# lturing/tacotronv2_wavernn_chinese

Measured on AMD Instinct MI355X. Metric: audio ksamples/sec (22.05 kHz, 10-bit RAW WaveRNN, batch=1 per GPU), higher is better.
Workload: dtype f32

## Files before the change

tacotronv2_wavernn_chinese_amd/csrc/loop_team2.hip:

```cpp
#include "team_common.h"

#define T2_THREADS 512

namespace {

template <int N>
__device__ __forceinline__ void peek_n(const u64 *base, unsigned idx, unsigned stride, u64 (&g)[N]) {
#pragma unroll
    for (int i = 0; i < N; ++i) g[i] = __hip_atomic_load(base + idx + (unsigned)i * stride, __ATOMIC_RELAXED, __HIP_MEMORY_SCOPE_AGENT);
}
template <int N, int SHIFT>
__device__ __forceinline__ bool tags_ok(const u64 (&g)[N], unsigned tag) {
    bool ok = true;
#pragma unroll
    for (int i = 0; i < N; ++i) ok = ok && ((unsigned)(g[i] >> SHIFT) == tag);
    return ok;
}
template <int N, int SHIFT>
__device__ __forceinline__ void finish_n(const u64 *base, unsigned idx, unsigned stride, unsigned tag, u64 (&g)[N], bool &dead,
                                         unsigned *err, unsigned code) {
    unsigned spins = 0;
    while (!dead && !__all(tags_ok<N, SHIFT>(g, tag))) {
        if (++spins > TEAM_SPIN_MAX) { dead = true; if ((threadIdx.x & 63) == 0) atomicExch(err, code); break; }
        peek_n<N>(base, idx, stride, g);
    }
}

#ifndef T2_HOIST_LDS
#define T2_HOIST_LDS 1
#endif
#ifndef T2_STRAIGHT_POLL
#define T2_STRAIGHT_POLL 7
#endif
#ifndef T2_DEFER_OUT
#define T2_DEFER_OUT 0
#endif
#ifndef T2_PRESLEEP
#define T2_PRESLEEP 0
#endif

__device__ __forceinline__ void hoist_fence() {
#if T2_HOIST_LDS
    __builtin_amdgcn_sched_barrier(0);
#endif
}
__device__ __forceinline__ void pin(float &v) {
#if T2_HOIST_LDS
    asm volatile("" : "+v"(v));
#endif
}

#if T2_STRAIGHT_POLL & 1
__device__ __forceinline__ unsigned take_granule(const u64 *base, unsigned idx, unsigned tag, bool &dead, unsigned *err, unsigned code) {
#if T2_PRESLEEP
    __builtin_amdgcn_s_sleep(T2_PRESLEEP);
#endif
    u64 g;
    for (unsigned spins = 0;;) {
        g = __hip_atomic_load(base + idx, __ATOMIC_RELAXED, __HIP_MEMORY_SCOPE_AGENT);
        if (__all((unsigned)(g >> 32) == tag) || dead) break;
        if (++spins > TEAM_SPIN_MAX) { dead = true; if ((threadIdx.x & 63) == 0) atomicExch(err, code); break; }
    }
    return (unsigned)g;
}
#else
__device__ __forceinline__ unsigned take_granule(const u64 *base, unsigned idx, unsigned tag, bool &dead, unsigned *err, unsigned code) {
    u64 ga[1];
#if T2_PRESLEEP
    __builtin_amdgcn_s_sleep(T2_PRESLEEP);
#endif
    peek_n<1>(base, idx, 1, ga);
    finish_n<1, 32>(base, idx, 1, tag, ga, dead, err, code);
    return (unsigned)ga[0];
}
#endif

__device__ __forceinline__ float rows_max(float v) {
    asm volatile(
        "s_nop 1\n\t"
        "v_max_f32_dpp %0, %0, %0 row_bcast:15 row_mask:0xa bank_mask:0xf\n\t"
        "s_nop 1\n\t"
        "v_max_f32_dpp %0, %0, %0 row_bcast:31 row_mask:0xc bank_mask:0xf\n\t"
        "s_nop 1"
        : "+v"(v));
    return v;
}

typedef unsigned u4 __attribute__((ext_vector_type(4)));
#ifndef T2_RACE_SLEEP
#define T2_RACE_SLEEP 3
#endif
__device__ __forceinline__ u4 race_load(const u64 *base, unsigned off) {
    u4 g;
    asm volatile("global_load_dwordx4 %0, %1, %2 sc1\n\t"
                 "s_waitcnt vmcnt(0)"
                 : "=&v"(g) : "v"(off), "s"(base) : "memory");
    return g;
}
__device__ __forceinline__ bool race_ok(const u4 &g, unsigned tag) { return (g.y >> 10) == tag && (g.w >> 10) == tag; }

#define XB_PLANE 68
#define XB_VEC (8 * XB_PLANE)
__device__ __forceinline__ int perm(int j) { return ((j >> 2) & 7) * XB_PLANE + (j >> 5) * 4 + (j & 3); }

typedef float f2 __attribute__((ext_vector_type(2)));
__device__ __forceinline__ f2 mk2(float a, float b) { f2 r; r.x = a; r.y = b; return r; }
__device__ __forceinline__ f2 pkfma(f2 a, f2 b, f2 c) { return __builtin_elementwise_fma(a, b, c); }

__device__ __forceinline__ void dot32x3(const float *w, const float *vec, int q, float &o0, float &o1, float &o2) {
    const float4 *p = (const float4 *)vec + q;
    f2 a = mk2(0.f, 0.f), b = mk2(0.f, 0.f), c = mk2(0.f, 0.f);
#pragma unroll
    for (int h = 0; h < 2; ++h) {
        float4 x[4];
#pragma unroll
        for (int k = 0; k < 4; ++k) x[k] = p[(4 * h + k) * (XB_PLANE / 4)];
#pragma unroll
        for (int k = 0; k < 4; ++k) {
            const int kk = 4 * h + k;
            const f2 xl = mk2(x[k].x, x[k].y), xh = mk2(x[k].z, x[k].w);
            a = pkfma(mk2(w[4 * kk + 0], w[4 * kk + 1]), xl, a);
            b = pkfma(mk2(w[32 + 4 * kk + 0], w[32 + 4 * kk + 1]), xl, b);
            c = pkfma(mk2(w[64 + 4 * kk + 0], w[64 + 4 * kk + 1]), xl, c);
            a = pkfma(mk2(w[4 * kk + 2], w[4 * kk + 3]), xh, a);
            b = pkfma(mk2(w[32 + 4 * kk + 2], w[32 + 4 * kk + 3]), xh, b);
            c = pkfma(mk2(w[64 + 4 * kk + 2], w[64 + 4 * kk + 3]), xh, c);
        }
    }
    o0 = a.x + a.y; o1 = b.x + b.y; o2 = c.x + c.y;
}
__device__ __forceinline__ void dot32x3_mixed(const float *w, const float4 *wl_, const float *vec, int q, float &o0, float &o1, float &o2) {
    const float4 *p = (const float4 *)vec + q;
    f2 a = mk2(0.f, 0.f), b = mk2(0.f, 0.f), c = mk2(0.f, 0.f);
#pragma unroll
    for (int h = 0; h < 2; ++h) {
        float4 x[4], wn[4];
#pragma unroll
        for (int k = 0; k < 4; ++k) { x[k] = p[(4 * h + k) * (XB_PLANE / 4)]; wn[k] = wl_[(4 * h + k) * 256]; }
#pragma unroll
        for (int k = 0; k < 4; ++k) {
            const int kk = 4 * h + k;
            const f2 xl = mk2(x[k].x, x[k].y), xh = mk2(x[k].z, x[k].w);
            a = pkfma(mk2(w[4 * kk + 0], w[4 * kk + 1]), xl, a);
            b = pkfma(mk2(w[32 + 4 * kk + 0], w[32 + 4 * kk + 1]), xl, b);
            c = pkfma(mk2(wn[k].x, wn[k].y), xl, c);
            a = pkfma(mk2(w[4 * kk + 2], w[4 * kk + 3]), xh, a);
            b = pkfma(mk2(w[32 + 4 * kk + 2], w[32 + 4 * kk + 3]), xh, b);
            c = pkfma(mk2(wn[k].z, wn[k].w), xh, c);
        }
    }
    o0 = a.x + a.y; o1 = b.x + b.y; o2 = c.x + c.y;
}
__device__ __forceinline__ float dot32(const float *w, const float *vec, int q) {
    const float4 *p = (const float4 *)vec + q;
    f2 s0 = mk2(0.f, 0.f), s1 = mk2(0.f, 0.f);
    float4 x[8];
#pragma unroll
    for (int k = 0; k < 8; ++k) x[k] = p[k * (XB_PLANE / 4)];
#pragma unroll
    for (int k = 0; k < 8; ++k) {
        s0 = pkfma(mk2(w[4 * k + 0], w[4 * k + 1]), mk2(x[k].x, x[k].y), s0);
        s1 = pkfma(mk2(w[4 * k + 2], w[4 * k + 3]), mk2(x[k].z, x[k].w), s1);
    }
    return (s0.x + s0.y) + (s1.x + s1.y);
}

constexpr int L_COND = 0;
constexpr int L_CSTA = L_COND + 512 * 4;
constexpr int L_GH1 = L_CSTA + 512 * 4;
constexpr int L_CSTQ = L_GH1 + 1536;
constexpr int L_HAND = L_CSTQ + 256;
constexpr int L_MISC = L_HAND + 128;
constexpr int L_XB = L_MISC + 64;
constexpr int XB_H1 = 0, XB_X2 = 1, XB_X3 = 2, XB_H2 = 3, XB_F1 = 4, XB_F2 = 5;
constexpr int L_SW = L_XB + 6 * XB_VEC;
constexpr int L_FC3 = L_SW + 8 * 256 * 4;
constexpr int L_XTAB = L_FC3 + 16384;
constexpr int L_TOTAL = L_XTAB + 1024;
static_assert(L_TOTAL * 4 <= 163840, "LDS budget");
constexpr int M_XF = 9;

constexpr unsigned G_X3 = 0, G_F1 = 1024, G_F2 = 2048, G_PR = 3072, G_GH = 4096;

}

#define P2(i)                                                               \
    do {                                                                    \
        if (PROF) {                                                         \
            const u64 now_ = __builtin_readcyclecounter();                  \
            prof_acc[i] += now_ - prof_last;                                \
            prof_last = now_;                                               \
        }                                                                   \
    } while (0)

template <int MODE, bool PROF, bool RAGGED>
__global__ void __launch_bounds__(T2_THREADS, 2) loop_team2_kernel(WrnnTeamArgs a) {
    extern __shared__ __attribute__((aligned(16))) char smem[];
    float *lds = (float *)smem;
    float *xb = lds + L_XB;
    float *gh1s = lds + L_GH1;
    int *misc_i = (int *)(lds + L_MISC);
    float *misc_f = lds + L_MISC;

    const int tid = threadIdx.x;
    const int lane = tid & 63, wave = __builtin_amdgcn_readfirstlane(tid >> 6);
    const bool isC = wave < 4;
    const int wl = wave & 3;
    if (isC) __builtin_amdgcn_s_setprio(3);
    const int r4 = lane >> 4, q = lane & 15;
    const WrnnDims d = a.d;
    const int NC = d.NC, HOP = d.HOP, T = a.T;
    const float4 *swl = (const float4 *)(lds + L_SW) + (tid - 256);

    int team, g;
    if (!join_team(a.ctl, a.err, misc_i, a.n_teams, team, g) || team >= a.n_rows) return;
    u64 *mail = a.mail + (size_t)team * WRNN_TEAM_MAIL_GRANULES;

    const int unit = 16 * g + 4 * wl + r4;
    const int qslot = wl * 4 + r4;
    const int c3row0 = 32 * g + 8 * wl + 2 * r4;
    const bool has_fc3 = c3row0 < NC;

    float wv[160];
    {
        const float *src = a.team_w + (size_t)g * WRNN_TEAM_NWREG * WRNN_TEAM_THREADS + (wl * 64 + lane);
        if (isC) {
#pragma unroll
            for (int i = 0; i < 96; ++i) wv[i] = src[(size_t)(96 + i) * WRNN_TEAM_THREADS];
#pragma unroll
            for (int i = 0; i < 64; ++i) wv[96 + i] = src[(size_t)(288 + i) * WRNN_TEAM_THREADS];
        } else {
#pragma unroll
            for (int i = 0; i < 96; ++i) wv[i] = src[(size_t)i * WRNN_TEAM_THREADS];
#pragma unroll
            for (int i = 0; i < 64; ++i) wv[96 + i] = src[(size_t)(192 + i) * WRNN_TEAM_THREADS];
#pragma unroll
            for (int k = 0; k < 8; ++k)
                ((float4 *)(lds + L_SW))[k * 256 + (tid - 256)] =
                    make_float4(src[(size_t)(256 + 4 * k) * WRNN_TEAM_THREADS], src[(size_t)(257 + 4 * k) * WRNN_TEAM_THREADS],
                                src[(size_t)(258 + 4 * k) * WRNN_TEAM_THREADS], src[(size_t)(259 + 4 * k) * WRNN_TEAM_THREADS]);
        }
        const float4 *f3 = (const float4 *)(a.team_fc3 + (size_t)g * 16384);
        float4 *dst = (float4 *)(lds + L_FC3);
        for (int i = tid; i < 4096; i += T2_THREADS) dst[i] = f3[i];
        if (MODE == WRNN_MODE_RAW)
            for (int k = tid; k < 1024; k += T2_THREADS) lds[L_XTAB + k] = 2.0f * (float)k / ((float)NC - 1.0f) - 1.0f;
        ((float4 *)(lds + L_CSTA))[tid] = make_float4(a.wI0[tid], a.u1[tid], a.u1[512 + tid], a.u1[1024 + tid]);
        if (!isC && q == 0) {
            float *cq = lds + L_CSTQ + qslot * 16;
            cq[0] = a.w[a.off.r1_bhh + unit]; cq[1] = a.w[a.off.r1_bhh + 512 + unit]; cq[2] = a.w[a.off.r1_bhh + 1024 + unit];
            cq[3] = a.w[a.off.r2_bhh + unit]; cq[4] = a.w[a.off.r2_bhh + 512 + unit]; cq[5] = a.w[a.off.r2_bhh + 1024 + unit];
            cq[6] = has_fc3 ? a.w[a.off.fc3_b + c3row0] : 0.0f;
            cq[7] = (c3row0 + 1 < NC) ? a.w[a.off.fc3_b + c3row0 + 1] : 0.0f;
        }
    }
    __syncthreads();
    float *cstQ = lds + L_CSTQ + qslot * 16;
    float *hand = lds + L_HAND + qslot * 8;
    const int pj = perm(tid), pu = perm(unit);
    const int sidx = tid - 256;

    bool dead = false;
    unsigned epoch = 0;
    u64 prof_acc[17] = {0};
    u64 prof_last = 0;

    for (int it = team; it < (RAGGED ? a.n_slots : a.n_rows); it += a.n_teams) {
        int row = it;
        if constexpr (RAGGED) {
            row = a.sched[it];
            if (row < 0) continue;
        }
        const WrnnRow rw = a.rows[row];
        uint64_t kseed = a.seed;
        uint32_t krow = (uint32_t)row;
        if (a.keys) { const WrnnRowKey k = a.keys[row]; kseed = k.seed; krow = k.row; }
        int64_t seg_end = a.seg0 + a.seg_len;
        if constexpr (RAGGED) {
            if (a.seg0 >= rw.steps) continue;
            if (seg_end > rw.steps) seg_end = rw.steps;
        }
        const bool resume = a.seg0 > 0;
        float *st = a.state + (size_t)row * WRNN_TEAM_STATE_FLOATS;
        const float4 *CONDg = (const float4 *)a.tabCOND + ((size_t)row * a.seg_len - (size_t)a.seg0) * 512;
        const float *C2g = a.tabC2 + (size_t)rw.utt * (T + 1) * 1536;
        const float *C3g = a.tabC3 + (size_t)rw.utt * (T + 1) * 512;
        const float *C4g = a.tabC4 + (size_t)rw.utt * (T + 1) * 512;

        float h1_j = resume ? st[tid] : 0.0f;
        float xfeed = resume ? st[4096] : (a.x_init ? a.x_init[row] : 0.0f);
        xb[XB_H2 * XB_VEC + pj] = resume ? st[512 + tid] : 0.0f;
        for (int i = tid; i < 1536; i += T2_THREADS) gh1s[i] = resume ? st[1024 + i] : a.w[a.off.r1_bhh + i];
        if (tid == 0) misc_f[M_XF] = xfeed;
        const int64_t pos0 = rw.start + a.seg0;
        int nfi = (int)(pos0 / HOP), nph = (int)(pos0 - (int64_t)nfi * HOP);
        int cst_frame = -1000000;
        int pend_frame = -1;
        float nzE0 = 0.f, nzE1 = 0.f, nzn0 = 0.f, nzn1 = 0.f;
        float4 cnext0 = make_float4(0.f, 0.f, 0.f, 0.f), cnext1 = cnext0;

        auto s_prepare = [&](int64_t ts, unsigned ep_of_ts) {
            const bool live = nfi < T;
            const int fi = live ? nfi : T;
            if (++nph == HOP) { nph = 0; ++nfi; }
            pend_frame = fi;
            ((float4 *)(lds + L_COND))[sidx] = cnext0;
            ((float4 *)(lds + L_COND))[sidx + 256] = cnext1;
        };
        auto s_prefetch = [&](int64_t ts) {
            if (ts < seg_end) {
                const float4 *cp = CONDg + (size_t)ts * 512;
                const unsigned so = (unsigned)sidx & 255u;
                cnext0 = cp[so];
                cnext1 = cp[256 + so];
            }
        };
        auto s_noise = [&](int64_t ts, unsigned ep_of_ts) {
            if (MODE == WRNN_MODE_MOL && wave == 4 && lane <= NC / 3) {
                const int nr = NC / 3;
                float u;
                if (a.noise_mode == WRNN_NOISE_INJECTED)
                    u = lane < nr ? a.noise1[((size_t)ts * a.n_rows + row) * nr + lane] : a.noise2[(size_t)ts * a.n_rows + row];
                else
                    u = wrnn_uniform_mol(kseed, (uint64_t)ts, krow, (uint32_t)lane);
                misc_f[32 + 16 * (ep_of_ts & 1u) + lane] = lane < nr ? -logf(-logf(u)) : logf(u) - logf(1.0f - u);
            }
            if (MODE == WRNN_MODE_RAW && has_fc3) {
                float nz0 = 0.f, nz1 = 0.f;
                if (a.noise_mode == WRNN_NOISE_INJECTED) {
                    const float *qp = a.noise1 + ((size_t)ts * a.n_rows + row) * NC + c3row0;
                    nz0 = -logf(qp[0]); nz1 = -logf(qp[1]);
                    if (q == 0) { hand[4 + 2 * (ep_of_ts & 1u)] = nz0; hand[5 + 2 * (ep_of_ts & 1u)] = nz1; }
                } else if (a.noise_mode == WRNN_NOISE_PHILOX) {
                    if ((ts & 31) == 0) {
                        const Philox4 pz = wrnn_raw_block(kseed, (uint64_t)ts + 2u * (unsigned)q, krow, (uint32_t)c3row0);
                        nzE0 = -__logf(-logf(u01_from_bits(pz.x)));
                        nzE1 = -__logf(-logf(u01_from_bits(pz.y)));
                        nzn0 = -__logf(-logf(u01_from_bits(pz.z)));
                        nzn1 = -__logf(-logf(u01_from_bits(pz.w)));
                    }
                    if (q == (int)((ts >> 1) & 15)) {
                        const bool odd = (ts & 1) != 0;
                        hand[4 + 2 * (ep_of_ts & 1u)] = odd ? nzn0 : nzE0;
                        hand[5 + 2 * (ep_of_ts & 1u)] = odd ? nzn1 : nzE1;
                    }
                } else if (q == 0) { hand[4 + 2 * (ep_of_ts & 1u)] = 0.f; hand[5 + 2 * (ep_of_ts & 1u)] = 0.f; }
            }
        };
        auto s_frame_consts = [&]() {
            if (pend_frame >= 0 && pend_frame != cst_frame) {
                if (q == 0) {
                    const int fi = pend_frame;
                    cstQ[8] = C2g[(size_t)fi * 1536 + unit]; cstQ[9] = C2g[(size_t)fi * 1536 + 512 + unit];
                    cstQ[10] = C2g[(size_t)fi * 1536 + 1024 + unit];
                    cstQ[11] = C3g[(size_t)fi * 512 + unit];
                    cstQ[12] = C4g[(size_t)fi * 512 + unit];
                }
                cst_frame = __builtin_amdgcn_readfirstlane(pend_frame);
            }
        };
        if (!isC) {
            if (q == 0) {
                hand[0] = resume ? st[2560 + unit] : cstQ[3];
                hand[1] = resume ? st[2560 + 512 + unit] : cstQ[4];
                hand[2] = resume ? st[2560 + 1024 + unit] : cstQ[5];
            }
            s_prefetch(a.seg0);
            s_prepare(a.seg0, epoch + 1);
            s_prefetch(a.seg0 + 1);
            s_noise(a.seg0, epoch + 1);
            s_frame_consts();
        }
        __syncthreads();

        int out_k = 0;
        float out_x = 0.0f;
        for (int64_t t = a.seg0; t < seg_end; ++t) {
            ++epoch;
            const unsigned par = epoch & 1u;
            if (PROF) prof_last = __builtin_readcyclecounter();

            float x2_j;
            {
                const float4 cA = ((const float4 *)(lds + L_CSTA))[tid];
                const float4 cd = ((const float4 *)(lds + L_COND))[tid];
                const float ghr = gh1s[tid], ghz = gh1s[512 + tid], ghn = gh1s[1024 + tid];
                const float xprev = xfeed;
                const float xin = fmaf(cA.x, xprev, cd.x);
                const float rg = sigmoid_fast(fmaf(cA.y, xprev, cd.y) + ghr);
                const float zg = sigmoid_fast(fmaf(cA.z, xprev, cd.z) + ghz);
                const float ng = tanh_fast(fmaf(cA.w, xprev, cd.w) + rg * ghn);
                h1_j = (1.0f - zg) * ng + zg * h1_j;
                x2_j = xin + h1_j;
                xb[XB_H1 * XB_VEC + pj] = h1_j;
                xb[XB_X2 * XB_VEC + pj] = x2_j;
            }
            P2(0);
            __syncthreads();
            P2(1);

            if (isC) {
                float h2o = xb[XB_H2 * XB_VEC + pu];
                float x2u = xb[XB_X2 * XB_VEC + pu];
                float g2r = hand[0], g2z = hand[1], g2n = hand[2];
                float c2r = cstQ[8], c2z = cstQ[9], c2n = cstQ[10];
                hoist_fence();
                float gr, gz, gn;
                dot32x3(wv, xb + XB_X2 * XB_VEC, q, gr, gz, gn);
                pin(h2o); pin(x2u); pin(g2r); pin(g2z); pin(g2n); pin(c2r); pin(c2z); pin(c2n);
                gr = row_sum(gr) + c2r; gz = row_sum(gz) + c2z; gn = row_sum(gn) + c2n;
                const float rg = sigmoid_fast(gr + g2r);
                const float zg = sigmoid_fast(gz + g2z);
                const float ng = tanh_fast(gn + rg * g2n);
                const float x3u = x2u + ((1.0f - zg) * ng + zg * h2o);
                if (q == 0) st_granule(mail, G_X3 + par * 512 + unit, epoch, __float_as_uint(x3u));
            } else {
                if (T2_DEFER_OUT && MODE == WRNN_MODE_RAW && g == 0 && tid == 256 && t > a.seg0) {
                    if (a.labels_out) a.labels_out[(size_t)row * a.steps + t - 1] = out_k;
                    a.samples_out[(size_t)row * a.steps + t - 1] = out_x;
                }
                float sr, sz, sn;
                __builtin_amdgcn_s_sleep(2);
                float b1r = cstQ[0], b1z = cstQ[1], b1n = cstQ[2];
                hoist_fence();
                dot32x3(wv, xb + XB_H1 * XB_VEC, q, sr, sz, sn);
                pin(b1r); pin(b1z); pin(b1n);
                sr = row_sum(sr) + b1r; sz = row_sum(sz) + b1z; sn = row_sum(sn) + b1n;
                if (q == 0) {
                    st_granule(mail, G_GH + par * 1536 + unit, epoch, __float_as_uint(sr));
                    st_granule(mail, G_GH + par * 1536 + 512 + unit, epoch, __float_as_uint(sz));
                    st_granule(mail, G_GH + par * 1536 + 1024 + unit, epoch, __float_as_uint(sn));
                }
            }
            P2(2);
            {
                const float x3 = __uint_as_float(take_granule(mail, G_X3 + par * 512 + tid, epoch, dead, a.err, 11u));
                xb[XB_X3 * XB_VEC + pj] = x3;
                xb[XB_H2 * XB_VEC + pj] = x3 - x2_j;
            }
            P2(3);
            __syncthreads();
            P2(4);

            if (isC) {
                float c3u = cstQ[11];
                hoist_fence();
                const float d = dot32(wv + 128, xb + XB_X3 * XB_VEC, q);
                pin(c3u);
                const float s = row_sum(d) + c3u;
                if (q == 0) st_granule(mail, G_F1 + par * 512 + unit, epoch, __float_as_uint(fmaxf(s, 0.0f)));
            } else {
                if (t + 1 < seg_end) s_noise(t + 1, epoch + 1);
            }
            P2(5);
            {
                xb[XB_F1 * XB_VEC + pj] = __uint_as_float(take_granule(mail, G_F1 + par * 512 + tid, epoch, dead, a.err, 12u));
            }
            P2(6);
            __syncthreads();
            P2(7);

            if (isC) {
                float c4u = cstQ[12];
                hoist_fence();
                const float d = dot32(wv + 96, xb + XB_F1 * XB_VEC, q);
                pin(c4u);
                const float s = row_sum(d) + c4u;
                if (q == 0) st_granule(mail, G_F2 + par * 512 + unit, epoch, __float_as_uint(fmaxf(s, 0.0f)));
            } else {
                if (t + 1 < seg_end) s_prepare(t + 1, epoch + 1);
            }
            P2(8);
            {
                xb[XB_F2 * XB_VEC + pj] = __uint_as_float(take_granule(mail, G_F2 + par * 512 + tid, epoch, dead, a.err, 13u));
            }
            P2(9);
            __syncthreads();
            P2(10);

            if (isC) {
                float lg0, lg1;
#if T2_HOIST_LDS
                float b3a = cstQ[6], b3b = cstQ[7];
                float2 nz = make_float2(0.f, 0.f);
                if (MODE == WRNN_MODE_RAW) nz = *(const float2 *)(hand + 4 + 2 * par);
                hoist_fence();
#endif
                {
                    const float4 *xp = (const float4 *)(xb + XB_F2 * XB_VEC) + q;
                    const float4 *wp = (const float4 *)(lds + L_FC3) + (size_t)(wl * 2) * 8 * 64 + lane;
                    f2 pa = mk2(0.f, 0.f), pb = mk2(0.f, 0.f);
#pragma unroll
                    for (int kk = 0; kk < 8; kk += 4) {
                        float4 x[4], wa[4], wb[4];
#pragma unroll
                        for (int k = 0; k < 4; ++k) { x[k] = xp[(kk + k) * (XB_PLANE / 4)]; wa[k] = wp[(kk + k) * 64]; wb[k] = wp[(8 + kk + k) * 64]; }
#pragma unroll
                        for (int k = 0; k < 4; ++k) {
                            const f2 xl = mk2(x[k].x, x[k].y), xh = mk2(x[k].z, x[k].w);
                            pa = pkfma(mk2(wa[k].x, wa[k].y), xl, pa); pb = pkfma(mk2(wb[k].x, wb[k].y), xl, pb);
                            pa = pkfma(mk2(wa[k].z, wa[k].w), xh, pa); pb = pkfma(mk2(wb[k].z, wb[k].w), xh, pb);
                        }
                    }
#if T2_HOIST_LDS
                    pin(b3a); pin(b3b); pin(nz.x); pin(nz.y);
                    lg0 = row_sum(pa.x + pa.y) + b3a;
                    lg1 = row_sum(pb.x + pb.y) + b3b;
#else
                    lg0 = row_sum(pa.x + pa.y) + cstQ[6];
                    lg1 = row_sum(pb.x + pb.y) + cstQ[7];
#endif
                }
                if (a.logits_out && q == 0 && has_fc3) {
                    int c3o = c3row0;
                    asm volatile("" : "+v"(c3o));
                    float *lo = a.logits_out + ((size_t)t * a.n_rows + row) * NC + c3o;
                    lo[0] = lg0;
                    if (c3row0 + 1 < NC) lo[1] = lg1;
                }
                if (MODE == WRNN_MODE_RAW) {
#if T2_HOIST_LDS
                    const float v0 = has_fc3 ? lg0 + nz.x : -INFINITY;
                    const float v1 = (c3row0 + 1 < NC) ? lg1 + nz.y : -INFINITY;
#else
                    const float v0 = has_fc3 ? lg0 + hand[4 + 2 * par] : -INFINITY;
                    const float v1 = (c3row0 + 1 < NC) ? lg1 + hand[5 + 2 * par] : -INFINITY;
#endif
                    const bool p1 = v1 > v0;
                    const float bq = p1 ? v1 : v0;
                    const int kq = p1 ? c3row0 + 1 : c3row0;
                    const float mw = __int_as_float(__builtin_amdgcn_readlane(__float_as_int(rows_max(bq)), 63));
                    const u64 bw = __ballot(bq == mw);
                    const int kw = __builtin_amdgcn_readlane(kq, (int)__builtin_ctzll(bw ? bw : 1ull));
                    if (lane == 0) st_granule(mail, G_PR + par * 512 + 4 * g + wl, (epoch << 10) | (unsigned)kw, __float_as_uint(mw));
                    P2(13);
                    if (wave == 0) {
                        if (T2_RACE_SLEEP) __builtin_amdgcn_s_sleep(T2_RACE_SLEEP);
                        const unsigned roff = (G_PR + par * 512 + 2u * (unsigned)lane) * 8u;
                        const unsigned rtag = epoch & 0x3fffffu;
#if T2_STRAIGHT_POLL & 2
                        u4 gq;
                        for (unsigned spins = 0;;) {
                            gq = race_load(mail, roff);
                            if (__all(race_ok(gq, rtag)) || dead) break;
                            if (++spins > TEAM_SPIN_MAX) { dead = true; if (lane == 0) atomicExch(a.err, 14u); break; }
                        }
#else
                        u4 gq = race_load(mail, roff);
                        for (unsigned spins = 0; !dead && !__all(race_ok(gq, rtag));) {
                            if (++spins > TEAM_SPIN_MAX) { dead = true; if (lane == 0) atomicExch(a.err, 14u); break; }
                            gq = race_load(mail, roff);
                        }
#endif
                        P2(14);
                        const float va = __uint_as_float(gq.x), vb = __uint_as_float(gq.z);
                        const bool pb_ = vb > va;
                        const float best = pb_ ? vb : va;
                        const int besti = (int)((pb_ ? gq.w : gq.y) & 1023u);
                        const float bestx = lds[L_XTAB + besti];
                        const float mx = __int_as_float(__builtin_amdgcn_readlane(__float_as_int(wave_max(best)), 63));
                        const u64 ball = __ballot(best == mx);
                        const int src = (int)__builtin_ctzll(ball ? ball : 1ull);
                        if (lane == 0) {
                            misc_i[16] = __builtin_amdgcn_readlane(__float_as_int(bestx), src);
                            misc_i[17] = __builtin_amdgcn_readlane(besti, src);
                        }
                    }
                } else {
                    if (q == 0 && has_fc3) {
                        st_granule(mail, G_PR + par * 512 + c3row0, epoch, __float_as_uint(lg0));
                        if (c3row0 + 1 < NC) st_granule(mail, G_PR + par * 512 + c3row0 + 1, epoch, __float_as_uint(lg1));
                    }
                    if (wave == 0) {
                        const int nr = NC / 3;
                        float mylg = 0.0f;
                        if (lane < NC) {
                            u64 gq[1];
                            peek_n<1>(mail, G_PR + par * 512 + lane, 1, gq);
                            unsigned spins = 0;
                            while (!dead && (unsigned)(gq[0] >> 32) != epoch) {
                                if (++spins > TEAM_SPIN_MAX) { dead = true; atomicExch(a.err, 16u); break; }
                                peek_n<1>(mail, G_PR + par * 512 + lane, 1, gq);
                            }
                            mylg = __uint_as_float((unsigned)gq[0]);
                        }
                        const float v = lane < nr ? mylg + misc_f[32 + 16 * par + lane] : -INFINITY;
                        const float mx = __int_as_float(__builtin_amdgcn_readlane(__float_as_int(wave_max(v)), 63));
                        const u64 ball = __ballot(v == mx);
                        const int km = (int)__builtin_ctzll(ball ? ball : 1ull);
                        const float mean = __int_as_float(__builtin_amdgcn_readlane(__float_as_int(mylg), nr + km));
                        const float ls = fmaxf(__int_as_float(__builtin_amdgcn_readlane(__float_as_int(mylg), 2 * nr + km)), -32.23619130191664f);
                        float xs = mean + expf(ls) * misc_f[32 + 16 * par + nr];
                        xs = fminf(fmaxf(xs, -1.0f), 1.0f);
                        if (lane == 0) {
                            float xf = xs;
                            if (a.x_forced) { float v = a.x_forced[(size_t)t * a.n_rows + row]; asm volatile("" : "+v"(v)); xf = v; }
                            misc_f[M_XF] = xf;
                            if (g == 0) {
                                if (a.labels_out) a.labels_out[(size_t)row * a.steps + t] = km;
                                a.samples_out[(size_t)row * a.steps + t] = xs;
                            }
                        }
                    }
                }
            } else {
                s_frame_consts();
                s_prefetch(t + 2);
#if T2_STRAIGHT_POLL & 4
                u64 gq[6];
                for (unsigned spins = 0;;) {
                    peek_n<6>(mail, G_GH + par * 1536 + sidx, 256, gq);
                    if (__all(tags_ok<6, 32>(gq, epoch)) || dead) break;
                    if (++spins > TEAM_SPIN_MAX) { dead = true; if (lane == 0) atomicExch(a.err, 15u); break; }
                }
#else
                u64 gq[6];
                peek_n<6>(mail, G_GH + par * 1536 + sidx, 256, gq);
                finish_n<6, 32>(mail, G_GH + par * 1536 + sidx, 256, epoch, gq, dead, a.err, 15u);
#endif
#pragma unroll
                for (int m = 0; m < 6; ++m) gh1s[sidx + m * 256] = __uint_as_float((unsigned)gq[m]);
                P2(13);
                {
                    float sr, sz, sn;
                    float b2r = cstQ[3], b2z = cstQ[4], b2n = cstQ[5];
                    hoist_fence();
                    dot32x3_mixed(wv + 96, swl, xb + XB_H2 * XB_VEC, q, sr, sz, sn);
                    pin(b2r); pin(b2z); pin(b2n);
                    sr = row_sum(sr) + b2r; sz = row_sum(sz) + b2z; sn = row_sum(sn) + b2n;
                    if (q == 0) { hand[0] = sr; hand[1] = sz; hand[2] = sn; }
                }
            }
            P2(11);
            __syncthreads();
            P2(12);
            if (MODE == WRNN_MODE_RAW) {
                const float2 win = *(const float2 *)(misc_f + 16);
                const float x_new = win.x;
                const int bk = __float_as_int(win.y);
                P2(15);
                xfeed = x_new;
                if (a.x_forced) { float v = a.x_forced[(size_t)t * a.n_rows + row]; asm volatile("" : "+v"(v)); xfeed = v; }
                out_k = bk; out_x = x_new;
#if !T2_DEFER_OUT
                if (g == 0 && tid == 0) {
                    if (a.labels_out) a.labels_out[(size_t)row * a.steps + t] = bk;
                    a.samples_out[(size_t)row * a.steps + t] = x_new;
                }
#endif
            } else {
                xfeed = misc_f[M_XF];
            }
            if ((t & 63) == 63) {
                if (dead && lane == 0) misc_i[M_DEAD] = 1;
                __syncthreads();
                if (misc_i[M_DEAD]) return;
            }
        }
        __syncthreads();
        if (T2_DEFER_OUT && MODE == WRNN_MODE_RAW && g == 0 && tid == 256 && seg_end > a.seg0) {
            if (a.labels_out) a.labels_out[(size_t)row * a.steps + seg_end - 1] = out_k;
            a.samples_out[(size_t)row * a.steps + seg_end - 1] = out_x;
        }
        if (seg_end < (RAGGED ? (int64_t)a.rows[row].steps : a.steps)) {
            if (g == 0) {
                st[tid] = h1_j;
                st[512 + tid] = xb[XB_H2 * XB_VEC + pj];
                for (int i = tid; i < 1536; i += T2_THREADS) st[1024 + i] = gh1s[i];
                if (tid == 0) st[4096] = xfeed;
            }
            if (!isC && q == 0) { st[2560 + unit] = hand[0]; st[2560 + 512 + unit] = hand[1]; st[2560 + 1024 + unit] = hand[2]; }
        }
    }
    if (PROF && a.prof && lane == 0 && g == 0 && team == 0) {
        for (int i = 0; i < 17; ++i) a.prof[wave * WRNN_PROF_SLOTS + i] += prof_acc[i];
    }
}

static const void *team2_fn(int mode, bool prof, bool ragged) {
    if (mode == WRNN_MODE_RAW) {
        if (ragged) return (const void *)loop_team2_kernel<WRNN_MODE_RAW, false, true>;
        return prof ? (const void *)loop_team2_kernel<WRNN_MODE_RAW, true, false> : (const void *)loop_team2_kernel<WRNN_MODE_RAW, false, false>;
    }
    return ragged ? (const void *)loop_team2_kernel<WRNN_MODE_MOL, false, true> : (const void *)loop_team2_kernel<WRNN_MODE_MOL, false, false>;
}

hipError_t wrnn_team2_occupancy(int mode, bool prof, int *blocks_per_cu, size_t *lds_bytes) {
    const size_t lds = (size_t)L_TOTAL * sizeof(float);
    *lds_bytes = lds;
    int worst = 1 << 30;
    for (int ragged = 0; ragged < 2; ++ragged) {
        const void *fn = team2_fn(mode, prof, ragged != 0);
        hipError_t e = hipFuncSetAttribute(fn, hipFuncAttributeMaxDynamicSharedMemorySize, (int)lds);
        if (e != hipSuccess) return e;
        int blocks = 0;
        e = hipOccupancyMaxActiveBlocksPerMultiprocessor(&blocks, fn, T2_THREADS, lds);
        if (e != hipSuccess) return e;
        if (blocks < worst) worst = blocks;
    }
    *blocks_per_cu = worst;
    return hipSuccess;
}

hipError_t wrnn_launch_loop_team2(const WrnnTeamArgs &a, hipStream_t s) {
    (void)hipGetLastError();
    const size_t lds = (size_t)L_TOTAL * sizeof(float);
    const bool ragged = a.ragged != 0, prof = a.prof != nullptr && a.d.mode == WRNN_MODE_RAW && !ragged;
    const void *fn = team2_fn(a.d.mode, prof, ragged);
    hipError_t e = hipFuncSetAttribute(fn, hipFuncAttributeMaxDynamicSharedMemorySize, (int)lds);
    if (e != hipSuccess) return e;
    void *args[] = {(void *)&a};
    return hipLaunchKernel(fn, dim3(a.n_teams * 32), dim3(T2_THREADS), args, lds, s);
}
```

Baseline: 320.9.

## Hoist step-head LDS reads to loop tail and shadow output stores on helper wave

Moves the per-step LDS reads of gate constants, conditioning and GRU-1 hidden contributions, plus the phase-B operands, into a single batch at the end of the previous iteration, so they are issued before the loop back-edge. Sample and label global stores move from thread 0 on the critical compute waves to a helper-wave thread, which writes the previous step's output from LDS during its noise slot. It also hides Philox operands from the optimizer with an empty asm. The risks are higher register pressure at two blocks per CU and reading LDS state one step early, which relies on the existing barriers to keep the values consistent.

```diff
diff --git a/tacotronv2_wavernn_chinese_amd/csrc/loop_team2.hip b/tacotronv2_wavernn_chinese_amd/csrc/loop_team2.hip
--- a/tacotronv2_wavernn_chinese_amd/csrc/loop_team2.hip
+++ b/tacotronv2_wavernn_chinese_amd/csrc/loop_team2.hip
@@ -32,8 +32,17 @@
 #ifndef T2_STRAIGHT_POLL
 #define T2_STRAIGHT_POLL 7
 #endif
-#ifndef T2_DEFER_OUT
-#define T2_DEFER_OUT 0
+#ifndef T2_HEAD_ONE_TRIP
+#define T2_HEAD_ONE_TRIP 1
+#endif
+#ifndef T2_OUT_SHADOW
+#define T2_OUT_SHADOW 1
+#endif
+#ifndef T2_PREB1_OPERANDS
+#define T2_PREB1_OPERANDS 1
+#endif
+#ifndef T2_PHILOX_OPAQUE
+#define T2_PHILOX_OPAQUE 1
 #endif
 #ifndef T2_PRESLEEP
 #define T2_PRESLEEP 0
@@ -193,6 +202,31 @@
         }                                                                   \
     } while (0)
 
+#define T2_PHASE_A_READS()                                                  \
+    do {                                                                    \
+        hA = ((const float4 *)(lds + L_CSTA))[tid];                         \
+        hD = ((const float4 *)(lds + L_COND))[tid];                         \
+        hgr = gh1s[tid]; hgz = gh1s[512 + tid]; hgn = gh1s[1024 + tid];     \
+    } while (0)
+#if T2_PREB1_OPERANDS
+#define T2_PHASE_B_READS()                                                  \
+    do {                                                                    \
+        pq0 = cstQ[8]; pq1 = cstQ[9]; pq2 = cstQ[10];                       \
+        pg0 = hand[0]; pg1 = hand[1]; pg2 = hand[2];                        \
+        ph2 = xb[XB_H2 * XB_VEC + pu];                                      \
+    } while (0)
+#else
+#define T2_PHASE_B_READS() do { } while (0)
+#endif
+#define T2_HEAD_READS() do { __builtin_amdgcn_sched_barrier(0); T2_PHASE_A_READS(); __builtin_amdgcn_sched_barrier(0); T2_PHASE_B_READS(); __builtin_amdgcn_sched_barrier(0); } while (0)
+#define T2_STORE_OUT(ts)                                                                                    \
+    do {                                                                                                    \
+        const float2 win_ = *(const float2 *)(misc_f + 16);                                                 \
+        if (a.labels_out) a.labels_out[(size_t)row * a.steps + (ts)] = __float_as_int(win_.y);              \
+        a.samples_out[(size_t)row * a.steps + (ts)] = win_.x;                                               \
+    } while (0)
+#define T2_OUT_THREAD (T2_OUT_SHADOW && MODE == WRNN_MODE_RAW && g == 0 && tid == 256)
+
 template <int MODE, bool PROF, bool RAGGED>
 __global__ void __launch_bounds__(T2_THREADS, 2) loop_team2_kernel(WrnnTeamArgs a) {
     extern __shared__ __attribute__((aligned(16))) char smem[];
@@ -333,7 +367,11 @@
                     if (q == 0) { hand[4 + 2 * (ep_of_ts & 1u)] = nz0; hand[5 + 2 * (ep_of_ts & 1u)] = nz1; }
                 } else if (a.noise_mode == WRNN_NOISE_PHILOX) {
                     if ((ts & 31) == 0) {
-                        const Philox4 pz = wrnn_raw_block(kseed, (uint64_t)ts + 2u * (unsigned)q, krow, (uint32_t)c3row0);
+                        int c3p = c3row0, qp = q;
+#if T2_PHILOX_OPAQUE
+                        asm volatile("" : "+v"(c3p), "+v"(qp));
+#endif
+                        const Philox4 pz = wrnn_raw_block(kseed, (uint64_t)ts + 2u * (unsigned)qp, krow, (uint32_t)c3p);
                         nzE0 = -__logf(-logf(u01_from_bits(pz.x)));
                         nzE1 = -__logf(-logf(u01_from_bits(pz.y)));
                         nzn0 = -__logf(-logf(u01_from_bits(pz.z)));
@@ -373,8 +411,12 @@
         }
         __syncthreads();
 
-        int out_k = 0;
-        float out_x = 0.0f;
+        float4 hA = make_float4(0.f, 0.f, 0.f, 0.f), hD = hA;
+        float hgr = 0.f, hgz = 0.f, hgn = 0.f;
+        float pq0 = 0.f, pq1 = 0.f, pq2 = 0.f, pg0 = 0.f, pg1 = 0.f, pg2 = 0.f, ph2 = 0.f;
+#if T2_HEAD_ONE_TRIP
+        T2_HEAD_READS();
+#endif
         for (int64_t t = a.seg0; t < seg_end; ++t) {
             ++epoch;
             const unsigned par = epoch & 1u;
@@ -382,9 +424,11 @@
 
             float x2_j;
             {
-                const float4 cA = ((const float4 *)(lds + L_CSTA))[tid];
-                const float4 cd = ((const float4 *)(lds + L_COND))[tid];
-                const float ghr = gh1s[tid], ghz = gh1s[512 + tid], ghn = gh1s[1024 + tid];
+#if !T2_HEAD_ONE_TRIP
+                T2_HEAD_READS();
+#endif
+                const float4 cA = hA, cd = hD;
+                const float ghr = hgr, ghz = hgz, ghn = hgn;
                 const float xprev = xfeed;
                 const float xin = fmaf(cA.x, xprev, cd.x);
                 const float rg = sigmoid_fast(fmaf(cA.y, xprev, cd.y) + ghr);
@@ -400,10 +444,14 @@
             P2(1);
 
             if (isC) {
+                float x2u = xb[XB_X2 * XB_VEC + pu];
+#if T2_PREB1_OPERANDS
+                float h2o = ph2, g2r = pg0, g2z = pg1, g2n = pg2, c2r = pq0, c2z = pq1, c2n = pq2;
+#else
                 float h2o = xb[XB_H2 * XB_VEC + pu];
-                float x2u = xb[XB_X2 * XB_VEC + pu];
                 float g2r = hand[0], g2z = hand[1], g2n = hand[2];
                 float c2r = cstQ[8], c2z = cstQ[9], c2n = cstQ[10];
+#endif
                 hoist_fence();
                 float gr, gz, gn;
                 dot32x3(wv, xb + XB_X2 * XB_VEC, q, gr, gz, gn);
@@ -415,10 +463,6 @@
                 const float x3u = x2u + ((1.0f - zg) * ng + zg * h2o);
                 if (q == 0) st_granule(mail, G_X3 + par * 512 + unit, epoch, __float_as_uint(x3u));
             } else {
-                if (T2_DEFER_OUT && MODE == WRNN_MODE_RAW && g == 0 && tid == 256 && t > a.seg0) {
-                    if (a.labels_out) a.labels_out[(size_t)row * a.steps + t - 1] = out_k;
-                    a.samples_out[(size_t)row * a.steps + t - 1] = out_x;
-                }
                 float sr, sz, sn;
                 __builtin_amdgcn_s_sleep(2);
                 float b1r = cstQ[0], b1z = cstQ[1], b1n = cstQ[2];
@@ -450,6 +494,7 @@
                 const float s = row_sum(d) + c3u;
                 if (q == 0) st_granule(mail, G_F1 + par * 512 + unit, epoch, __float_as_uint(fmaxf(s, 0.0f)));
             } else {
+                if (T2_OUT_THREAD && t > a.seg0) T2_STORE_OUT(t - 1);
                 if (t + 1 < seg_end) s_noise(t + 1, epoch + 1);
             }
             P2(5);
@@ -635,14 +680,20 @@
             __syncthreads();
             P2(12);
             if (MODE == WRNN_MODE_RAW) {
+#if T2_OUT_SHADOW
+                const float x_new = misc_f[16];
+#else
                 const float2 win = *(const float2 *)(misc_f + 16);
                 const float x_new = win.x;
                 const int bk = __float_as_int(win.y);
+#endif
+#if T2_HEAD_ONE_TRIP
+                T2_HEAD_READS();
+#endif
                 P2(15);
                 xfeed = x_new;
                 if (a.x_forced) { float v = a.x_forced[(size_t)t * a.n_rows + row]; asm volatile("" : "+v"(v)); xfeed = v; }
-                out_k = bk; out_x = x_new;
-#if !T2_DEFER_OUT
+#if !T2_OUT_SHADOW
                 if (g == 0 && tid == 0) {
                     if (a.labels_out) a.labels_out[(size_t)row * a.steps + t] = bk;
                     a.samples_out[(size_t)row * a.steps + t] = x_new;
@@ -650,18 +701,21 @@
 #endif
             } else {
                 xfeed = misc_f[M_XF];
+#if T2_HEAD_ONE_TRIP
+                T2_HEAD_READS();
+#endif
             }
             if ((t & 63) == 63) {
                 if (dead && lane == 0) misc_i[M_DEAD] = 1;
                 __syncthreads();
-                if (misc_i[M_DEAD]) return;
+                if (misc_i[M_DEAD]) {
+                    if (T2_OUT_THREAD) T2_STORE_OUT(t);
+                    return;
+                }
             }
         }
         __syncthreads();
-        if (T2_DEFER_OUT && MODE == WRNN_MODE_RAW && g == 0 && tid == 256 && seg_end > a.seg0) {
-            if (a.labels_out) a.labels_out[(size_t)row * a.steps + seg_end - 1] = out_k;
-            a.samples_out[(size_t)row * a.steps + seg_end - 1] = out_x;
-        }
+        if (T2_OUT_THREAD && seg_end > a.seg0) T2_STORE_OUT(seg_end - 1);
         if (seg_end < (RAGGED ? (int64_t)a.rows[row].steps : a.steps)) {
             if (g == 0) {
                 st[tid] = h1_j;
```

After: 329.5 (median of 6 runs). +2.7%, better.
